# MuellerNico/DD2360-RayTracing

Measured on AMD Instinct MI355X. Metric: Msamples/s (W*H*spp/render_time) at 1200x800, 10000 spheres, higher is better.
Workload: dtype f32

## Files before the change

dd2360-raytracing_amd/csrc/rt_kernels.hip:

```cpp
#include <hip/hip_runtime.h>
#include <float.h>
#include "rt_device.h"
#include "rt_tuning.h"
#include "rt_sampling.h"
#include "rt_sched_keep.h"

#ifdef RT_TU_CONTRACT
#pragma clang fp contract(fast)
#else
#pragma clang fp contract(off)
#endif

namespace rt {
#ifdef RT_TU_CONTRACT
namespace fmac {
#endif

#define RT_DEV static __device__ __forceinline__

#include "rt_stats.h"

struct Rng { uint32_t d, v0, v1, v2, v3, v4; };

RT_DEV float rng_uniform(Rng& s) {
    const uint32_t t = s.v0 ^ (s.v0 >> 2);
    s.v0 = s.v1; s.v1 = s.v2; s.v2 = s.v3; s.v3 = s.v4;
    s.v4 = (s.v4 ^ (s.v4 << 4)) ^ (t ^ (t << 1));
    s.d += 362437u;
    return uniform_from_bits(s.d + s.v4);
}

RT_DEV void rng_seed(Rng& s, unsigned long long seed) {
    const uint32_t lo = (uint32_t)seed ^ 0xaad26b49u, hi = (uint32_t)(seed >> 32) ^ 0xf7dcefddu;
    const uint32_t t0 = 1099087573u * lo, t1 = 2591861531u * hi;
    s.d = 6615241u + t1 + t0;
    s.v0 = 123456789u + t0; s.v1 = 362436069u ^ t0; s.v2 = 521288629u + t1; s.v3 = 88675123u ^ t1; s.v4 = 5783321u + t0;
}

struct V3 { float x, y, z; };
RT_DEV float dot3(const V3& a, const V3& b) { return a.x * b.x + a.y * b.y + a.z * b.z; }

struct RayF { V3 o, d; };

RT_DEV float pow5(float x) { const double v = (double)x; const double v2 = v * v; return (float)((v2 * v2) * v); }

RT_DEV void sphere_test(const RayF& r, float a, float cx, float cy, float cz, float r2, int id, float& closest, int& best) {
    const float ocx = r.o.x - cx, ocy = r.o.y - cy, ocz = r.o.z - cz;
    const float b = ocx * r.d.x + ocy * r.d.y + ocz * r.d.z;
    const float c = (ocx * ocx + ocy * ocy + ocz * ocz) - r2;
    const float disc = b * b - a * c;
    if (disc > 0.0f) {
        const float sq = sqrtf(disc);
        float t = (-b - sq) / a;
        if (t < closest && t > 0.001f) { closest = t; best = id; }
        else {
            t = (-b + sq) / a;
            if (t < closest && t > 0.001f) { closest = t; best = id; }
        }
    }
}

RT_DEV bool ray_box(const RayF& r, float lox, float loy, float loz, float hix, float hiy, float hiz) {
    float tmin = (lox - r.o.x) / r.d.x;
    float tmax = (hix - r.o.x) / r.d.x;
    if (tmin > tmax) { const float t = tmin; tmin = tmax; tmax = t; }
    float tymin = (loy - r.o.y) / r.d.y;
    float tymax = (hiy - r.o.y) / r.d.y;
    if (tymin > tymax) { const float t = tymin; tymin = tymax; tymax = t; }
    if ((tmin > tymax) || (tymin > tmax)) return false;
    if (tymin > tmin) tmin = tymin;
    if (tymax < tmax) tmax = tymax;
    float tzmin = (loz - r.o.z) / r.d.z;
    float tzmax = (hiz - r.o.z) / r.d.z;
    if (tzmin > tzmax) { const float t = tzmin; tzmin = tzmax; tzmax = t; }
    if ((tmin > tzmax) || (tzmin > tmax)) return false;
    return true;
}

RT_DEV const RenderArgs* cold_args() {
    auto p = __builtin_amdgcn_kernarg_segment_ptr();
    asm volatile("" : "+s"(p));
    return (const RenderArgs*)p;
}

RT_DEV float bcast(float v, int l) { return __int_as_float(__builtin_amdgcn_readlane(__float_as_int(v), l)); }
template <int LG>
RT_DEV float group_min(float v) {
    const int inf = 0x7f800000;
    int x = __float_as_int(v);
#define RT_DPP_MIN(ctrl, rmask) x = __float_as_int(fminf(__int_as_float(x), __int_as_float(__builtin_amdgcn_update_dpp(inf, x, ctrl, rmask, 0xf, false))))
    RT_DPP_MIN(0x111, 0xf);
    RT_DPP_MIN(0x112, 0xf);
    RT_DPP_MIN(0x114, 0xf);
    RT_DPP_MIN(0x118, 0xf);
    if (LG >= 32) RT_DPP_MIN(0x142, 0xa);
    if (LG >= 64) RT_DPP_MIN(0x143, 0xc);
#undef RT_DPP_MIN
    const int q3 = __builtin_amdgcn_readlane(x, 63);
    if (LG == 64) return __int_as_float(q3);
    const int q1 = __builtin_amdgcn_readlane(x, 31);
    if (LG == 32) return __int_as_float((threadIdx.x & 32) ? q3 : q1);
    const int q0 = __builtin_amdgcn_readlane(x, 15), q2 = __builtin_amdgcn_readlane(x, 47);
    const int g = (threadIdx.x >> 4) & 3;
    return __int_as_float(g == 0 ? q0 : g == 1 ? q1 : g == 2 ? q2 : q3);
}
RT_DEV int wave_min_int(int x) {
    const int big = 0x7fffffff;
#define RT_DPP_MIN(ctrl, rmask) x = min(x, __builtin_amdgcn_update_dpp(big, x, ctrl, rmask, 0xf, false))
    RT_DPP_MIN(0x111, 0xf); RT_DPP_MIN(0x112, 0xf); RT_DPP_MIN(0x114, 0xf); RT_DPP_MIN(0x118, 0xf); RT_DPP_MIN(0x142, 0xa); RT_DPP_MIN(0x143, 0xc);
#undef RT_DPP_MIN
    return __builtin_amdgcn_readlane(x, 63);
}
RT_DEV int bcast(int v, int l) { return __builtin_amdgcn_readlane(v, l); }

RT_DEV float sphere_candidate(const RayF& r, float a, const float4 s) {
    const float ocx = r.o.x - s.x, ocy = r.o.y - s.y, ocz = r.o.z - s.z;
    const float b = ocx * r.d.x + ocy * r.d.y + ocz * r.d.z;
    const float c = (ocx * ocx + ocy * ocy + ocz * ocz) - s.w;
    const float disc = b * b - a * c;
    float cand = __builtin_inff();
    if (disc > 0.0f) {
        const float sq = sqrtf(disc);
        const float t1 = (-b - sq) / a;
        if (t1 > 0.001f) cand = t1;
        else {
            const float t2 = (-b + sq) / a;
            if (t2 > 0.001f) cand = t2;
        }
    }
    return cand;
}

RT_DEV void closest_list(const DevScene& S, const RayF& r, float a, bool live, float& closest, int& best) {
    const float4* __restrict__ hot = S.list_hot;
    const int n = S.n_list;
    unsigned long long todo = __ballot(live);
    if ((int)__popcll(todo) * RT_LIST_COOP_COST <= n) {
        const int lane = threadIdx.x & 63;
        while (todo != 0ull) {
            const int L = __ffsll((long long)todo) - 1;
            todo &= todo - 1ull;
            RayF q;
            q.o.x = bcast(r.o.x, L); q.o.y = bcast(r.o.y, L); q.o.z = bcast(r.o.z, L);
            q.d.x = bcast(r.d.x, L); q.d.y = bcast(r.d.y, L); q.d.z = bcast(r.d.z, L);
            const float qa = bcast(a, L);
            float my_t = FLT_MAX; int my_k = 0x7fffffff;
            for (int base = 0; base < n; base += 256) {
                float4 sv[4];
#pragma unroll
                for (int u = 0; u < 4; ++u) { const int k = base + u * 64 + lane; sv[u] = hot[k < n ? k : n - 1]; }
#pragma unroll
                for (int u = 0; u < 4; ++u) {
                    const int k = base + u * 64 + lane;
                    if (k < n) {
                        const float cand = sphere_candidate(q, qa, sv[u]);
                        if (cand < my_t) { my_t = cand; my_k = k; }
                    }
// ... 554 lines not shown
                bool anyhold = false;
#pragma unroll
                for (int k = 0; k < PB; ++k) {
                    const float ocx = S.q.o.x - s4[k].x, ocy = S.q.o.y - s4[k].y, ocz = S.q.o.z - s4[k].z;
                    const float b = ocx * S.q.d.x + ocy * S.q.d.y + ocz * S.q.d.z;
                    const float c = (ocx * ocx + ocy * ocy + ocz * ocz) - s4[k].w;
                    const float disc = b * b - S.a * c;
                    const float ab = fabsf(b);
                    const float Lm = __builtin_fmaf(ab, -1e-4f, -b) - S.abt, M = __builtin_fmaf(ab, -1e-4f, b) + S.atm;
                    const float P = fmaxf(Lm, M);
                    hold[k] = (unsigned)k < nb && disc > 0.0f && !(P > 0.0f && P * P > disc * 1.0003f);
                    hb[k] = b; hd[k] = disc;
                    anyhold = anyhold || hold[k];
                }
                if (__ballot(anyhold) != 0ull) {
#pragma unroll
                    for (int k = 0; k < PB; ++k) {
                        const unsigned long long hm = __ballot(hold[k]);
                        if (hm != 0ull) {
                            const unsigned slot = qn + __builtin_amdgcn_mbcnt_hi((unsigned)(hm >> 32), __builtin_amdgcn_mbcnt_lo((unsigned)hm, 0u));
                            if (hold[k]) {
                                STAT(st, ST_DISCPOS, 1);
                                const uint4 ce = make_uint4(__float_as_uint(hb[k]), __float_as_uint(hd[k]), he0 + (unsigned)k, (unsigned)S.owner);
                                if (slot < (unsigned)kWalkCand) L.cq[slot] = ce;
                                else pool_candidate(T, s_nodes, L, ce STAT_PASS);
                            }
                            qn += (unsigned)__popcll(hm);
                        }
                    }
                }
                S.cur += nb;
                if (qn >= (unsigned)RT_DENSE_DRAIN) pool_drain(T, s_nodes, L, lane, qn STAT_PASS);
            }
            pool_drain(T, s_nodes, L, lane, qn STAT_PASS);
            const unsigned long long k = L.key[lane];
            best_t = __uint_as_float((unsigned)(k >> 32)); best = (int)(unsigned)k;
            const unsigned tmask = lane < 32 ? L.tie_lo : L.tie_hi;
            if ((tmask >> (lane & 31)) & 1u) tie = true;
        }
        if (walking && best >= 0) walk_clip(W, A, best_t);
        walking = walking && W.i != W.iend;
        const int left = __popcll(__ballot(walking));
        if (left == 0) break;
        if (RT_QUORUM_DEN > 0 && nw0 >= RT_QUORUM_MIN && left * RT_QUORUM_DEN <= nw0) break;
    }
    W.walking = walking;
}

constexpr int kHotLarge = 8;
constexpr int kHotSlots = 1 + 3 * kHotLarge;
RT_DEV float4* hot_spheres(const float4* s_nodes, int n_nodes) { return (float4*)((WalkLds*)(s_nodes + n_nodes * 3) + 4); }
template <bool POOL>
RT_DEV void stage_tree_fp32(const DevScene& S, const DevTree& T, float4* s_nodes) {
    const int n4 = T.n_nodes * 3;
    for (int t = threadIdx.x; t < n4; t += 256) s_nodes[t] = T.nodes4[t];
    if (POOL) {
        float4* h = hot_spheres(s_nodes, T.n_nodes);
        const int nl = min(T.acc.n_large, kHotLarge);
        if (threadIdx.x == 0) h[0] = S.ground_valid ? S.list_hot[0] : make_float4(0.f, 0.f, 0.f, 0.f);
        if ((int)threadIdx.x < nl) h[1 + threadIdx.x] = T.acc.large_hot[threadIdx.x];
        if ((int)threadIdx.x < 2 * nl) h[1 + kHotLarge + threadIdx.x] = T.acc.large_brick[threadIdx.x];
    }
    __syncthreads();
}

struct TreeState { Walk W; float g_t; int g_id; bool tie, pending; unsigned work, cols; };
RT_DEV void tree_state_init(TreeState& ts) {
    ts.pending = false; ts.tie = false; ts.g_t = FLT_MAX; ts.g_id = -1; ts.work = 0u; ts.cols = 0u; ts.W.work = 0u; ts.W.cols = 0u;
    ts.W.walking = false; ts.W.i = 0; ts.W.iend = 0; ts.W.coff = 0; ts.W.om_c = 0.f; ts.W.on_c = 0.f; ts.W.slope = 0.f; ts.W.dm_c = 0.f; ts.W.fwd = true;
}

template <int COOPG>
RT_DEV void closest_tree(const DevScene& S, const DevTree& T, const float4* s_nodes, const RayF& r, float a, bool live, float& closest, int& best, TreeState& ts STAT_ARG) {
    const bool fresh = live && !ts.pending;
    STAT(st, ST_RAYS, fresh ? 1 : 0);
    if (fresh) { closest = FLT_MAX; best = -1; }
    if (S.ground_valid && fresh) {
        WPASS(WP_GROUND);
        const float4 g = COOPG != 1 ? hot_spheres(s_nodes, T.n_nodes)[0] : S.list_hot[0];
        int gb = -1;
        { const float ocx = r.o.x - g.x, ocy = r.o.y - g.y, ocz = r.o.z - g.z;
          const float b = ocx * r.d.x + ocy * r.d.y + ocz * r.d.z;
          const float c = (ocx * ocx + ocy * ocy + ocz * ocz) - g.w;
          if (__ballot(fresh && !(b > 0.0f && c > 0.0f)) != 0ull) sphere_test(r, a, g.x, g.y, g.z, g.w, 0, closest, gb); }
        if (gb == 0) best = 0;
    }
    RT_STATS_ONLY(
    const unsigned long long tG = TICK(); st.cyc[4] += tG;
    )
    bool slow = fresh;
    if (COOPG != 1 && T.acc.enabled) {
        const float zx = r.o.x, zy = r.o.y - 1.0f, zz = r.o.z;
        const bool fast = fresh && (a >= 9.094947e-13f) && (a <= 1.0995116e12f) && (r.d.x != 0.0f) && (r.d.z != 0.0f)
                          && (fabsf(r.d.y) >= 9.094947e-13f) && (zx * zx + zy * zy + zz * zz <= T.acc.zone2);
        slow = fresh && !fast;
        STAT(st, ST_FAST, fast ? 1 : 0); STAT(st, ST_SLOW, slow ? 1 : 0);
        if (fast) {
            ts.g_t = closest; ts.g_id = best; ts.tie = false;
            const float ra = __builtin_amdgcn_rcpf(a);
            for (int k = 0; k < T.acc.n_large; ++k) {
                const float4* hs = hot_spheres(s_nodes, T.n_nodes);
                const float4 sp = k < kHotLarge ? hs[1 + k] : T.acc.large_hot[k];
                WPASS(WP_LARGE_K);
                const float ocx = r.o.x - sp.x, ocy = r.o.y - sp.y, ocz = r.o.z - sp.z;
                const float b = ocx * r.d.x + ocy * r.d.y + ocz * r.d.z;
                const float c = (ocx * ocx + ocy * ocy + ocz * ocz) - sp.w;
                const float disc = b * b - a * c;
                if (disc > 0.0f) {
                    const float sqa = __builtin_amdgcn_sqrtf(disc);
                    const float m = 1e-4f * ((fabsf(b) + sqa) * ra) + 1e-6f;
                    const bool behind = (sqa - b) * ra + m < 0.001f;
                    const bool beyond = (-b - sqa) * ra - m > closest;
                    if (!behind && !beyond) {
                        WPASS(WP_LARGE_EXACT);
                        const float sq = sqrtf(disc);
                        float cand = __builtin_inff();
                        const float t1 = (-b - sq) / a;
                        if (t1 > 0.001f) cand = t1;
                        else { const float t2 = (-b + sq) / a; if (t2 > 0.001f) cand = t2; }
                        offer(T, s_nodes, r, cand, k < kHotLarge ? hs[1 + kHotLarge + 2 * k] : T.acc.large_brick[2 * k], k < kHotLarge ? hs[2 + kHotLarge + 2 * k] : T.acc.large_brick[2 * k + 1], closest, best, ts.tie STAT_PASS);
                    }
                }
            }
            WPASS(WP_SETUP);
            ts.W = walk_setup(T.acc, r, closest, best);
        }
        RT_STATS_ONLY(
        const unsigned long long tL = TICK(); st.cyc[5] += tL - tG;
        )
        const bool walker = fast || (live && ts.pending);
        const int nw = __popcll(__ballot(walker));
        if (nw > 0) {
            WalkLds& L = *((WalkLds*)(s_nodes + T.n_nodes * 3) + (threadIdx.x >> 6));
            Walk Wl = ts.W; Wl.walking = walker && ts.W.walking;
            float bt = walker ? closest : FLT_MAX; int bi = walker ? best : -1; bool tt = false;
            if (COOPG >= 4) walk_pool<RT_QUORUM_SPARSE>(T, s_nodes, L, r, a, Wl, bt, bi, tt STAT_PASS);
            else walk_pool_dense<RT_QUORUM_DENSE>(T, s_nodes, L, r, a, Wl, bt, bi, tt STAT_PASS);
            if (walker) { ts.work += Wl.work; ts.cols += Wl.cols; Wl.work = 0u; Wl.cols = 0u; ts.W = Wl; closest = bt; best = bi; ts.tie = ts.tie || tt; }
        }
        if (walker) {
            ts.pending = ts.W.walking;
            if (!ts.pending && ts.tie) { closest = ts.g_t; best = ts.g_id; slow = true; STAT(st, ST_TIE, 1); }
        }
    }
    RT_STATS_ONLY(
    const unsigned long long tS0 = TICK(); st.cyc[1] += tS0 - tG;
    )
    if (__ballot(slow) != 0ull) { WPASS(WP_SCAN); tree_scan(s_nodes, r, a, slow, closest, best); }
    RT_STATS_ONLY(
    st.cyc[3] += TICK() - tS0;
    )
}

RT_DEV V3 random_in_unit_sphere(Rng& s) {
    V3 p;
    do {
        WPASS(WP_REJ_ITER);
        const float x = rng_uniform(s); const float y = rng_uniform(s); const float z = rng_uniform(s);
        p.x = signed_unit(x); p.y = signed_unit(y); p.z = signed_unit(z);
    } while (p.x * p.x + p.y * p.y + p.z * p.z >= 1.0f);
    return p;
}

RT_DEV RayF primary_ray(const rt_camera& c, int i, int j, int max_x, int max_y, Rng& s) {
    const float u = ((float)i + rng_uniform(s)) / (float)max_x;
    const float v = ((float)j + rng_uniform(s)) / (float)max_y;
    float px, py;
    WPASS(WP_PRIMARY);
    do {
        WPASS(WP_DISK_ITER);
        const float x = rng_uniform(s); const float y = rng_uniform(s);
        px = signed_unit(x); py = signed_unit(y);
    } while (px * px + py * py + 0.0f >= 1.0f);
    const float rdx = c.lens_radius * px, rdy = c.lens_radius * py;
    RayF r;
    const float ox = rdx * c.u[0] + rdy * c.v[0], oy = rdx * c.u[1] + rdy * c.v[1], oz = rdx * c.u[2] + rdy * c.v[2];
    r.o.x = c.origin[0] + ox; r.o.y = c.origin[1] + oy; r.o.z = c.origin[2] + oz;
    r.d.x = (((c.lower_left_corner[0] + u * c.horizontal[0]) + v * c.vertical[0]) - c.origin[0]) - ox;
    r.d.y = (((c.lower_left_corner[1] + u * c.horizontal[1]) + v * c.vertical[1]) - c.origin[1]) - oy;
    r.d.z = (((c.lower_left_corner[2] + u * c.horizontal[2]) + v * c.vertical[2]) - c.origin[2]) - oz;
    return r;
}

RT_DEV bool scatter(const DevScene& S, int sphere, float t, RayF& r, V3& att, Rng& s) {
    const float4 g = S.shade[2 * sphere];
    const float4 m = S.shade[2 * sphere + 1];
    const int kind = S.kind8[sphere];
    V3 p, n;
    p.x = r.o.x + t * r.d.x; p.y = r.o.y + t * r.d.y; p.z = r.o.z + t * r.d.z;
    n.x = (p.x - g.x) / g.w; n.y = (p.y - g.y) / g.w; n.z = (p.z - g.z) / g.w;
    V3 q = {0.0f, 0.0f, 0.0f};
    WPASS(WP_SC_ANY);
    if (kind != RT_MAT_DIELECTRIC) q = random_in_unit_sphere(s);
    float len = 1.0f; V3 ud = {0.0f, 0.0f, 0.0f};
    if (kind != RT_MAT_LAMBERTIAN) {
        len = sqrtf(r.d.x * r.d.x + r.d.y * r.d.y + r.d.z * r.d.z);
        ud.x = r.d.x / len; ud.y = r.d.y / len; ud.z = r.d.z / len;
    }
    if (kind == RT_MAT_LAMBERTIAN) {
        WPASS(WP_SC_LAMB);
        const float tx = (p.x + n.x) + q.x, ty = (p.y + n.y) + q.y, tz = (p.z + n.z) + q.z;
        r.d.x = tx - p.x; r.d.y = ty - p.y; r.d.z = tz - p.z;
        r.o = p;
        att.x *= m.x; att.y *= m.y; att.z *= m.z;
        return true;
    }
    if (kind == RT_MAT_METAL) {
        WPASS(WP_SC_METAL);
        const float k = 2.0f * dot3(ud, n);
        const float rx = ud.x - k * n.x, ry = ud.y - k * n.y, rz = ud.z - k * n.z;
        r.d.x = rx + m.w * q.x; r.d.y = ry + m.w * q.y; r.d.z = rz + m.w * q.z;
        r.o = p;
        att.x *= m.x; att.y *= m.y; att.z *= m.z;
        return dot3(r.d, n) > 0.0f;
    }
    WPASS(WP_SC_DIEL);
    const float ri = m.w, inv_ri = m.x, r0sq = m.y, ri2 = m.z;
    const float dn = dot3(r.d, n);
    const float k = 2.0f * dn;
    const float rx = r.d.x - k * n.x, ry = r.d.y - k * n.y, rz = r.d.z - k * n.z;
    V3 on; float ni, cosine;
    if (dn > 0.0f) {
        on.x = -n.x; on.y = -n.y; on.z = -n.z; ni = ri;
        cosine = dn / len;
        cosine = sqrtf(1.0f - ri2 * (1.0f - cosine * cosine));
    } else {
        on = n; ni = inv_ri;
        cosine = -dn / len;
    }
    const V3 uv = ud;
    const float dt = dot3(uv, on);
    const float disc = 1.0f - ni * ni * (1.0f - dt * dt);
    float fx = 0.0f, fy = 0.0f, fz = 0.0f, reflect_prob;
    if (disc > 0.0f) {
        const float sq = sqrtf(disc);
        fx = ni * (uv.x - dt * on.x) - sq * on.x;
        fy = ni * (uv.y - dt * on.y) - sq * on.y;
        fz = ni * (uv.z - dt * on.z) - sq * on.z;
        const float r0 = r0sq;
        reflect_prob = r0 + (1.0f - r0) * pow5(1.0f - cosine);
    } else {
        reflect_prob = 1.0f;
    }
    r.o = p;
    if (rng_uniform(s) < reflect_prob) { r.d.x = rx; r.d.y = ry; r.d.z = rz; }
    else { r.d.x = fx; r.d.y = fy; r.d.z = fz; }
    return true;
}

RT_DEV V3 sky(const RayF& r, const V3& att) {
    WPASS(WP_SKY);
    const float len = sqrtf(r.d.x * r.d.x + r.d.y * r.d.y + r.d.z * r.d.z);
    const float uy = r.d.y / len;
    const float t = 0.5f * (uy + 1.0f);
    const float omt = 1.0f - t;
    V3 c;
    c.x = att.x * (omt + t * 0.5f);
    c.y = att.y * (omt + t * 0.7f);
    c.z = att.z * (omt + t * 1.0f);
    return c;
}

#ifndef RT_TU_LIST
__global__ __launch_bounds__(256) void k_render_init(rt_rand_state* rand_state, int max_x, int max_y, int tiles_x, int part, int nparts, long long begin, long long end, long long n_local_tiles) {
    const int lane = threadIdx.x & 63;
    const long long local_tile = (long long)blockIdx.x * 4 + (threadIdx.x >> 6);
    if (local_tile >= n_local_tiles) return;
    const long long tile = part_tile(local_tile, part, nparts, begin, end);
    const int tx = (int)(tile % tiles_x), ty = (int)(tile / tiles_x);
    const int i = tx * 8 + (lane & 7), j = ty * 8 + (lane >> 3);
    const bool inside = (i < max_x) && (j < max_y);
    const bool whole = part_whole(nparts, begin, end);
    if (whole && !inside) return;
    const long long idx = whole ? (long long)j * max_x + i : local_tile * 64 + lane;
    const int pixel_index = j * max_x + i;
    Rng s; rng_seed(s, 1984ull + (unsigned long long)(long long)pixel_index);
    rt_rand_state out;
    out.d = s.d; out.v[0] = s.v0; out.v[1] = s.v1; out.v[2] = s.v2; out.v[3] = s.v3; out.v[4] = s.v4;
    out.boxmuller_flag = 0; out.boxmuller_flag_double = 0; out.boxmuller_extra = 0.f; out.pad_ = 0; out.boxmuller_extra_double = 0.0;
    rand_state[idx] = out;
}
#endif

template <bool TREE, int MODE, int COOPG>
__global__ __launch_bounds__(256, RT_RENDER_WAVES) void k_render(RenderArgs A) {
    extern __shared__ float4 s_nodes[];
    if (TREE) stage_tree_fp32<COOPG != 1>(A.scene, A.tree, s_nodes);
    const int lane = threadIdx.x & 63;
    const long long n_slots = (MODE == 2 && A.ad_list) ? (long long)*A.ad_count : A.n_local_tiles * 64;
    const int ns = (MODE != 1) ? A.ns : 1;

    const long long n_waves = (long long)gridDim.x * 4;
    long long slot = 0;
    int i = 0, j = 0; long long idx = 0;
    unsigned int iters = 0;
    bool is_long = false;
    bool is_med = false;
    bool retired = false;
    bool thin = false;
    bool thin_counted = false;
    bool long_done = false;
    const unsigned int n_long_raw = A.long_list ? A.queue[2] : 0u, n_solo_raw = A.long_list ? A.queue[4] : 0u;
    const bool use_long = (n_long_raw + n_solo_raw) != 0u && (long long)(n_long_raw + n_solo_raw) * 64 <= n_slots;
    const unsigned int n_long = use_long ? n_long_raw : 0u, n_solo = use_long ? n_solo_raw : 0u;
    bool solo = false, solo_done = false;
    Rng s = {0, 0, 0, 0, 0, 0};
    V3 col = {0.0f, 0.0f, 0.0f};
    V3 att = {1.0f, 1.0f, 1.0f};
    float sum_l = 0.0f, sum_q = 0.0f;
    RayF r; r.o = {0.f, 0.f, 0.f}; r.d = {0.f, 1.f, 0.f};
    int sample = 0, depth = 0;
    bool live = false;
    RT_STATS_ONLY(
    unsigned int pix_iters = 0;
    unsigned long long pix_t0 = 0;
    )

    constexpr bool kChunked = MODE == 1;
    constexpr long long kProgOwn = RT_PROG_OWN;
    const long long first_free = (kChunked && kProgOwn > 0 && n_waves * kProgOwn <= n_slots) ? n_waves * kProgOwn : 0;
    long long pool_next = 0, pool_end = 0;
    if (kChunked && first_free > 0) { pool_next = ((long long)blockIdx.x * 4 + (threadIdx.x >> 6)) * kProgOwn; pool_end = pool_next + kProgOwn; }
    auto take_slot = [&]() -> long long {
        return first_free + (long long)atomicAdd(cold_args()->queue, 1u);
    };
    auto begin_pixel = [&]() {
        live = false;
        const RenderArgs& A = *cold_args();
#ifdef RT_ONLY_LANE
        if (lane != RT_ONLY_LANE) return;
#endif
        iters = 0; is_long = false; is_med = false;
        while (slot < n_slots) {
            if constexpr (MODE == 2) {
                if (A.ad_list) {
                    const unsigned int pid = A.ad_list[slot];
                    idx = (long long)pid;
                    if (part_whole(A.nparts, A.tile_begin, A.tile_end)) { i = (int)(pid % (unsigned int)A.max_x); j = (int)(pid / (unsigned int)A.max_x); }
                    else {
                        const long long tile = part_tile((long long)(pid >> 6), A.part, A.nparts, A.tile_begin, A.tile_end);
                        const int tx = (int)(tile % A.tiles_x), ty = (int)(tile / A.tiles_x);
                        i = tx * 8 + (int)(pid & 7u); j = ty * 8 + (int)((pid >> 3) & 7u);
                    }
                    live = true;
                    break;
                }
            }
            long long local_tile; int l;
            const long long tail0 = (MODE != 1 && A.tail_list) ? (long long)A.queue[kQueueThr + 2] : 0;
            const long long head = tail0 > 0 ? (long long)A.queue[kQueueThr + 3] : 0;
            if (tail0 > 0 && (slot < head || slot >= tail0 - 1 + head)) {
                const bool from_end = A.queue[kQueueThr + 5] != 0u;
                const long long n_tail = n_slots - (tail0 - 1);
                const long long k = slot < head ? (from_end ? n_tail - head + slot : slot) : (from_end ? slot - (tail0 - 1) - head : slot - (tail0 - 1));
                const unsigned int pid = A.tail_list[k];
                local_tile = (long long)(pid >> 6); l = (int)(pid & 63u);
            } else {
                constexpr int kIl = COOPG == 2 ? RT_INTERLEAVE_DENSE : (COOPG == 5 ? RT_INTERLEAVE_SOLO : RT_INTERLEAVE);
                static_assert(kIl > 0 && 64 % kIl == 0, "RT_INTERLEAVE, RT_INTERLEAVE_DENSE and RT_INTERLEAVE_SOLO must divide 64 (the tail starts on a multiple of 64 tiles)");
                const long long ms = slot - head;
                const long long blk = ms / (64 * kIl);
                const long long tiles_in_blk = (A.n_local_tiles - blk * kIl) < kIl ? (A.n_local_tiles - blk * kIl) : kIl;
                const long long within = ms % (64 * kIl);
                const long long rank = blk * kIl + within % tiles_in_blk;
                l = (int)(within / tiles_in_blk);
                local_tile = A.order ? (long long)A.order[rank] : rank;
            }
            const long long tile = part_tile(local_tile, A.part, A.nparts, A.tile_begin, A.tile_end);
            const int tx = (int)(tile % A.tiles_x), ty = (int)(tile / A.tiles_x);
            i = tx * 8 + (l & 7); j = ty * 8 + (l >> 3);
            const bool taken = use_long && A.long_flag[local_tile * 64 + l];
            if (i < A.max_x && j < A.max_y && !taken) {
                idx = part_whole(A.nparts, A.tile_begin, A.tile_end) ? (long long)j * A.max_x + i : local_tile * 64 + l;
                live = true;
                RT_STATS_ONLY(
                pix_t0 = __builtin_amdgcn_s_memrealtime();
                )
                break;
            }
            slot = take_slot();
        }
        if (!live) retired = true;
        if (live) {
            const rt_rand_state* st = A.rand_state + idx;
            s.d = st->d; s.v0 = st->v[0]; s.v1 = st->v[1]; s.v2 = st->v[2]; s.v3 = st->v[3]; s.v4 = st->v[4];
            col = {0.0f, 0.0f, 0.0f}; att = {1.0f, 1.0f, 1.0f}; sample = 0; depth = 0;
            if constexpr (MODE == 2) {
                sum_l = 0.0f; sum_q = 0.0f;
                if (A.ad_list) {
                    const float* f = (const float*)A.fb + idx * 3;
                    col.x = f[0]; col.y = f[1]; col.z = f[2]; sum_l = A.ad_sl[idx]; sum_q = A.ad_q[idx];
                }
            }
            r = primary_ray(A.scene.cam, i, j, A.max_x, A.max_y, s);
        }
    };
    auto begin_long_pixel = [&](bool from_solo) -> bool {
        if (!use_long || (from_solo ? solo_done : long_done)) return false;
        const RenderArgs& A = *cold_args();
        long long pid;
        if (from_solo) {
            const unsigned int h = atomicAdd(A.queue + 5, 1u);
            if (h >= n_solo) { solo_done = true; return false; }
            pid = (long long)A.long_list[n_slots - 1 - (long long)h];
        } else {
            const unsigned int h = atomicAdd(A.queue + 3, 1u);
            if (h >= n_long) { long_done = true; return false; }
            const unsigned int stride = n_long % 257u ? 257u : (n_long % 263u ? 263u : 269u);
            pid = (long long)A.long_list[(unsigned int)(((unsigned long long)h * stride) % n_long)];
        }
        const long long local_tile = pid >> 6;
        const int l = (int)(pid & 63);
        const long long tile = part_tile(local_tile, A.part, A.nparts, A.tile_begin, A.tile_end);
        const int tx = (int)(tile % A.tiles_x), ty = (int)(tile / A.tiles_x);
        i = tx * 8 + (l & 7); j = ty * 8 + (l >> 3);
        idx = part_whole(A.nparts, A.tile_begin, A.tile_end) ? (long long)j * A.max_x + i : pid;
        live = true; iters = 0; is_long = true;
        RT_STATS_ONLY(
        pix_t0 = __builtin_amdgcn_s_memrealtime();
        )
        const rt_rand_state* st = A.rand_state + idx;
        s.d = st->d; s.v0 = st->v[0]; s.v1 = st->v[1]; s.v2 = st->v[2]; s.v3 = st->v[3]; s.v4 = st->v[4];
        col = {0.0f, 0.0f, 0.0f}; att = {1.0f, 1.0f, 1.0f}; sample = 0; depth = 0;
        if constexpr (MODE == 2) { sum_l = 0.0f; sum_q = 0.0f; }
        r = primary_ray(A.scene.cam, i, j, A.max_x, A.max_y, s);
        return true;
    };
    auto end_pixel = [&]() {
        const RenderArgs& A = *cold_args();
        rt_rand_state* st_out = A.rand_state + idx;
        st_out->d = s.d; st_out->v[0] = s.v0; st_out->v[1] = s.v1; st_out->v[2] = s.v2; st_out->v[3] = s.v3; st_out->v[4] = s.v4;
        float* fb = (float*)A.fb + idx * 3;
        if constexpr (MODE == 2) {
            fb[0] = col.x; fb[1] = col.y; fb[2] = col.z;
            A.ad_sl[idx] = sum_l; A.ad_q[idx] = sum_q;
        } else if (MODE == 0) {
            const float k = (float)(1.0 / (double)(float)A.ns);
            col.x *= k; col.y *= k; col.z *= k;
            fb[0] = sqrtf(col.x); fb[1] = sqrtf(col.y); fb[2] = sqrtf(col.z);
            RT_STATS_ONLY(
            fb[0] = (float)pix_iters; fb[1] = (float)((__builtin_amdgcn_s_memrealtime() >> 4) & 0xffffffull); fb[2] = (float)((pix_t0 >> 4) & 0xffffffull);
            )
        } else {
            if (A.ns == 1) { fb[0] = col.x; fb[1] = col.y; fb[2] = col.z; }
            else { fb[0] += col.x; fb[1] += col.y; fb[2] += col.z; }
        }
    };
    RT_STATS_ONLY(
    Stats st; for (int q = 0; q < ST_N; ++q) st.c[q] = 0;
    for (int q = 0; q < 8; ++q) st.cyc[q] = 0;
    const unsigned long long tK0 = TICK(), rK0 = __builtin_amdgcn_s_memrealtime();
    unsigned int dbg_thin_iters = 0, dbg_long = 0;
    unsigned long long th[4] = {0, 0, 0, 0};
    unsigned long long dbg_thin_cyc = 0, dbg_thin_closest = 0, dbg_thin1_cyc = 0; unsigned int dbg_thin1_iters = 0; unsigned long long dbg_t_prev = TICK();
    )
    constexpr bool kSolo = TREE && COOPG == 5;
    if (kSolo && lane == 0 && begin_long_pixel(true)) solo = true;
    if (__ballot(live) == 0ull && lane < RT_LONG_PER_WAVE) begin_long_pixel(false);
    if (__ballot(live) != 0ull) { thin = true; __builtin_amdgcn_s_setprio(3); }

    const unsigned int thin_cap = (unsigned int)(n_waves / RT_THIN_CAP_DEN);
    float closest = FLT_MAX; int best = -1;
    TreeState ts; tree_state_init(ts);
    while (true) {
        const unsigned long long m_live = __ballot(live);
        const unsigned long long m_long = __ballot(live && is_long);
        if (!thin && m_long != 0ull) {
            unsigned int prev = 0;
            if (lane == 0) prev = atomicAdd(cold_args()->queue + 1, 1u);
            prev = __builtin_amdgcn_readfirstlane(prev);
            if (prev < thin_cap) { thin = true; thin_counted = true; __builtin_amdgcn_s_setprio(3); }
            else { if (lane == 0) atomicSub(cold_args()->queue + 1, 1u); is_long = false; }
        } else if (thin && m_long == 0ull) {
            thin = false; __builtin_amdgcn_s_setprio(0);
            if (thin_counted && lane == 0) atomicSub(A.queue + 1, 1u);
            thin_counted = false;
        }
        if (RT_MED_RATE > 0 && !thin) { if (__ballot(live && is_med) != 0ull) __builtin_amdgcn_s_setprio(1); else __builtin_amdgcn_s_setprio(0); }
        if (!thin) {
            if (kChunked) {
                const bool need = !live && !retired;
                const unsigned long long mneed = __ballot(need);
                if (mneed != 0ull) {
                    const long long n = (long long)__popcll(mneed);
                    const long long left = pool_end - pool_next;
                    const long long rank = (long long)__builtin_amdgcn_mbcnt_hi((unsigned)(mneed >> 32), __builtin_amdgcn_mbcnt_lo((unsigned)mneed, 0u));
                    long long fresh = 0;
                    if (n > left) {
                        unsigned int b = 0;
                        if (lane == 0) b = atomicAdd(cold_args()->queue, 64u);
                        fresh = first_free + (long long)__builtin_amdgcn_readfirstlane(b);
                    }
                    if (need) slot = rank < left ? pool_next + rank : fresh + (rank - left);
                    if (n > left) { pool_next = fresh + (n - left); pool_end = fresh + 64; } else pool_next += n;
                    if (need) begin_pixel();
                }
            } else if (!live && !retired) { slot = take_slot(); begin_pixel(); }
        }
        if (__ballot(live) == 0ull) break;
        (void)m_live;
        STAT(st, ST_LOOP_ITERS_WAVE, 1);
        RT_STATS_ONLY(
        { const unsigned long long now = TICK(); const int nl2 = __popcll(__ballot(live));
          if (thin) { ++dbg_thin_iters; dbg_thin_cyc += now - dbg_t_prev; if (nl2 <= 2) { ++dbg_thin1_iters; dbg_thin1_cyc += now - dbg_t_prev; } }
          dbg_t_prev = now; }
        )
        RT_STATS_ONLY(
        { const int nl = __popcll(__ballot(live)); STAT(st, nl >= 56 ? ST_LIVE_GE56 : nl >= 32 ? ST_LIVE_32 : nl >= 8 ? ST_LIVE_8 : ST_LIVE_LT8, 1);
          WPASS_CLASS(nl >= 56 ? 0 : nl >= 32 ? 1 : nl >= 8 ? 2 : 3); }
        )
        const float a = dot3(r.d, r.d);
        if (!TREE) { closest = FLT_MAX; best = -1; }
        RT_STATS_ONLY(
        const unsigned long long tC0 = TICK();
        const unsigned long long c4_ = st.cyc[4], c5_ = st.cyc[5], c1_ = st.cyc[1], c3_ = st.cyc[3];
        const bool thin12 = thin && __popcll(__ballot(live)) <= 2;
        )
        if (TREE) closest_tree<COOPG>(A.scene, A.tree, s_nodes, r, a, live, closest, best, ts STAT_PASS);
        else closest_list(A.scene, r, a, live, closest, best);
        RT_STATS_ONLY(
        const unsigned long long tC1 = TICK(); st.cyc[0] += tC1 - tC0; st.cyc[2] += tC0; if (thin) dbg_thin_closest += tC1 - tC0;
        if (TREE && thin12) { th[0] += (st.cyc[4] - c4_) - tC0; th[1] += st.cyc[5] - c5_; th[2] += (st.cyc[1] - c1_) - (st.cyc[5] - c5_); th[3] += st.cyc[3] - c3_; }
        if (live) { ++pix_iters; }
        )
        if (live && !(TREE && ts.pending)) {
            ++iters;
            bool done;
            float lum = 0.0f;
            if (best >= 0) {
                const bool cont = scatter(cold_args()->scene, best, closest, r, att, s);
                ++depth;
                done = !cont || depth >= 50;
            } else {
                const V3 c = sky(r, att);
                col.x += c.x; col.y += c.y; col.z += c.z;
                if constexpr (MODE == 2) lum = (c.x + c.y) + c.z;
                done = true;
            }
            if (done) {
                if constexpr (MODE == 2) { sum_l += lum; sum_q += lum * lum; }
                (void)lum;
                ++sample; depth = 0; att = {1.0f, 1.0f, 1.0f};
                if (sample < ns) {
                    { const RenderArgs& C = *cold_args(); r = primary_ray(C.scene.cam, i, j, C.max_x, C.max_y, s); }
                    bool now_long = false;
                    if ((sample & (RT_LONG_CHECK - 1)) == 0 && sample + 8 <= ns) {
                        const unsigned int long_thr = MODE != 1 ? cold_args()->queue[kQueueThr] : 0u;
                        now_long = iters >= (unsigned int)((COOPG == 2 ? RT_LONG_RATE_DENSE : RT_LONG_RATE) * sample) ||
                                   (long_thr != 0u && (unsigned long long)iters * (unsigned int)ns >= (unsigned long long)long_thr * (unsigned int)sample);
                    }
                    if (now_long) {
                        RT_STATS_ONLY(
                        if (!is_long) ++dbg_long;
                        )
                        is_long = true;
                    }
                    else if (RT_MED_RATE > 0 && (sample & 7) == 0 && iters >= (unsigned int)(RT_MED_RATE * sample)) is_med = true;
                } else {
                    WPASS(WP_ENDPIX);
                    end_pixel();
                    RT_STATS_ONLY(
                    pix_iters = 0;
                    )
                    STAT(st, ST_SWITCHES, 1);
                    live = false; is_long = false; is_med = false;
                    if (kSolo && solo && begin_long_pixel(true)) {  }
                    else if (lane < RT_LONG_PER_WAVE && begin_long_pixel(false)) { solo = false;  }
                }
            }
        }
    }

    RT_STATS_ONLY(
    for (int q = 0; q < ST_N; ++q) {
        const bool wave_level = (q == ST_LOOP_ITERS_WAVE || (q >= ST_LIVE_GE56 && q <= ST_LIVE_LT8));
        const bool lane_max = (q == ST_A_ITERS_WAVE || q == ST_B_ROUNDS_WAVE);
        if (lane_max) { int m = (int)st.c[q]; for (int off = 32; off > 0; off >>= 1) m = max(m, __shfl_xor(m, off)); if (lane == 0) atomicAdd(&g_stats[q], (unsigned long long)m); }
        else if (st.c[q] && (!wave_level || lane == 0)) atomicAdd(&g_stats[q], (unsigned long long)st.c[q]);
    }
    { int nl = (int)dbg_long; for (int off = 32; off > 0; off >>= 1) nl += __shfl_xor(nl, off); dbg_long = (unsigned int)nl; }
    if (lane == 0) {
        const long long wv = (long long)blockIdx.x * 4 + (threadIdx.x >> 6);
        if (wv < 8192) {
            g_wave_dbg[wv * 4 + 0] = __builtin_amdgcn_s_memrealtime();
            g_wave_dbg[wv * 4 + 1] = st.c[ST_LOOP_ITERS_WAVE]; g_wave_dbg[wv * 4 + 2] = dbg_thin_iters; g_wave_dbg[wv * 4 + 3] = dbg_long;
            atomicAdd(&g_stats[TH_GROUND], th[0]); atomicAdd(&g_stats[TH_LARGE_SETUP], th[1]); atomicAdd(&g_stats[TH_WALK], th[2]); atomicAdd(&g_stats[TH_SCAN], th[3]);
            atomicAdd(&g_stats[ST_SPARE0], dbg_thin_cyc); atomicAdd(&g_stats[ST_SPARE1], dbg_thin_closest); atomicAdd(&g_stats[ST_SPARE2], dbg_thin1_cyc); atomicAdd(&g_stats[ST_SPARE3], (unsigned long long)dbg_thin1_iters); atomicAdd(&g_stats[ST_SPARE4], (unsigned long long)dbg_thin_iters);
        }
        atomicAdd(&g_stats[ST_SAMPLES], 1ull);
        const unsigned long long tot = TICK() - tK0;
        atomicAdd(&g_stats[ST_CYC_TOTAL], tot);
        atomicAdd(&g_stats[ST_CYC_CLOSEST], st.cyc[0]); atomicAdd(&g_stats[ST_CYC_WALK_A], st.cyc[1]); atomicAdd(&g_stats[ST_CYC_WALK_B], st.cyc[4] - st.cyc[2]);
        atomicAdd(&g_stats[ST_CYC_SCAN], st.cyc[3]); atomicAdd(&g_stats[ST_CYC_SHADE], tot - st.cyc[0]); atomicAdd(&g_stats[ST_SPARE4 + 1], st.cyc[5]); atomicAdd(&g_stats[ST_SPARE4 + 2], st.cyc[6]);
        atomicAdd(&g_stats[ST_REALTIME], __builtin_amdgcn_s_memrealtime() - rK0);
    }
    )
}

#if !defined(RT_TU_LIST) && !defined(RT_TU_CONTRACT)
__device__ __forceinline__ bool adapt_rule(float S, float Q, int k, float rel_error, float floor_lum) {
    const float nk = (float)k;
    const float d = nk * Q - S * S;
    const float nf = nk * floor_lum;
    const float m = S > nf ? S : nf;
    const float tt = rel_error * rel_error;
    return rel_error > 0.f && d <= (tt * (nk - 1.f)) * (m * m);
}
__device__ __forceinline__ bool adapt_in_frame(long long t, const AdaptFrame& fr) {
    const long long tile = part_tile(t >> 6, fr.part, fr.nparts, fr.tile_begin, fr.tile_end);
    const int tx = (int)(tile % fr.tiles_x), ty = (int)(tile / fr.tiles_x);
    return tx * 8 + (int)(t & 7) < fr.max_x && ty * 8 + (int)((t >> 3) & 7) < fr.max_y;
}
__device__ __forceinline__ void adapt_append(bool active, unsigned int pid, unsigned int* list_out, unsigned int* count_out) {
    const unsigned long long mask = __ballot(active);
    if (mask != 0ull) {
        unsigned int base = 0;
        if ((threadIdx.x & 63) == 0) base = atomicAdd(count_out, (unsigned int)__popcll(mask));
        base = __shfl(base, 0);
        const unsigned int rank = __builtin_amdgcn_mbcnt_hi((unsigned)(mask >> 32), __builtin_amdgcn_mbcnt_lo((unsigned)mask, 0u));
        if (active) list_out[base + rank] = pid;
    }
}
template <bool KEEP>
__device__ __forceinline__ void adapt_check(float* __restrict__ fb, const float* __restrict__ sl, const float* __restrict__ q,
                                            const unsigned int* __restrict__ list_in, const unsigned int* __restrict__ count_in, long long n_all,
                                            unsigned int* __restrict__ list_out, unsigned int* __restrict__ count_out, int32_t* __restrict__ spp,
                                            int k, int last, float rel_error, float floor_lum, const AdaptFrame& fr, const AdaptState& keep) {
    const long long t = (long long)blockIdx.x * 256 + threadIdx.x;
    const long long n = count_in ? (long long)*count_in : n_all;
    bool active = false;
    unsigned int pid = 0;
    bool inside = true;
    if (!list_in && t < n && !part_whole(fr.nparts, fr.tile_begin, fr.tile_end)) {
        const long long tile = part_tile(t >> 6, fr.part, fr.nparts, fr.tile_begin, fr.tile_end);
        const int tx = (int)(tile % fr.tiles_x), ty = (int)(tile / fr.tiles_x);
        inside = tx * 8 + (int)(t & 7) < fr.max_x && ty * 8 + (int)((t >> 3) & 7) < fr.max_y;
    }
    if (t < n && inside) {
        pid = list_in ? list_in[t] : (unsigned int)t;
        bool stop = last != 0;
        if (!stop) stop = adapt_rule(sl[pid], q[pid], k, rel_error, floor_lum);
        if (stop) {
            float* f = fb + (size_t)pid * 3;
            const float kk = (float)(1.0 / (double)(float)k);
            if constexpr (KEEP) {
                float* s = keep.rgb + (size_t)pid * 3;
                s[0] = f[0]; s[1] = f[1]; s[2] = f[2];
                keep.k[pid] = k;
            }
            f[0] = sqrtf(f[0] * kk); f[1] = sqrtf(f[1] * kk); f[2] = sqrtf(f[2] * kk);
            if (spp) spp[pid] = k;
        } else {
            active = true;
        }
    }
    adapt_append(active, pid, list_out, count_out);
}
__global__ __launch_bounds__(256) void k_adapt_check(float* __restrict__ fb, const float* __restrict__ sl, const float* __restrict__ q,
                                                     const unsigned int* __restrict__ list_in, const unsigned int* __restrict__ count_in, long long n_all,
                                                     unsigned int* __restrict__ list_out, unsigned int* __restrict__ count_out, int32_t* __restrict__ spp,
                                                     int k, int last, float rel_error, float floor_lum, AdaptFrame fr) {
    adapt_check<false>(fb, sl, q, list_in, count_in, n_all, list_out, count_out, spp, k, last, rel_error, floor_lum, fr, AdaptState{});
}
__global__ __launch_bounds__(256) void k_adapt_check_keep(float* __restrict__ fb, AdaptState s,
                                                          const unsigned int* __restrict__ list_in, const unsigned int* __restrict__ count_in, long long n_all,
                                                          unsigned int* __restrict__ list_out, unsigned int* __restrict__ count_out, int32_t* __restrict__ spp,
                                                          int k, int last, float rel_error, float floor_lum, AdaptFrame fr) {
    adapt_check<true>(fb, s.sl, s.q, list_in, count_in, n_all, list_out, count_out, spp, k, last, rel_error, floor_lum, fr, s);
}

__global__ __launch_bounds__(256) void k_adapt_refine_seed(float* __restrict__ fb, AdaptState s, long long n_all, unsigned int* __restrict__ list_out,
                                                           unsigned int* __restrict__ count_out, int32_t* __restrict__ spp,
                                                           int max_spp, float rel_error, float floor_lum, AdaptFrame fr) {
    const long long t = (long long)blockIdx.x * 256 + threadIdx.x;
    bool active = false;
    const unsigned int pid = (unsigned int)t;
    if (t < n_all && (part_whole(fr.nparts, fr.tile_begin, fr.tile_end) || adapt_in_frame(t, fr))) {
        const int k = s.k[pid];
        const float* S = s.rgb + (size_t)pid * 3;
        float* f = fb + (size_t)pid * 3;
        if (k >= max_spp || adapt_rule(s.sl[pid], s.q[pid], k, rel_error, floor_lum)) {
            const float kk = (float)(1.0 / (double)(float)k);
            f[0] = sqrtf(S[0] * kk); f[1] = sqrtf(S[1] * kk); f[2] = sqrtf(S[2] * kk);
            if (spp) spp[pid] = k;
        } else {
            f[0] = S[0]; f[1] = S[1]; f[2] = S[2];
            active = true;
        }
    }
    adapt_append(active, pid, list_out, count_out);
}
__global__ __launch_bounds__(256) void k_adapt_refine_check(float* __restrict__ fb, AdaptState s,
                                                            const unsigned int* __restrict__ list_in, const unsigned int* __restrict__ count_in,
                                                            unsigned int* __restrict__ list_out, unsigned int* __restrict__ count_out, int32_t* __restrict__ spp,
                                                            int batch, int max_spp, float rel_error, float floor_lum) {
    const long long t = (long long)blockIdx.x * 256 + threadIdx.x;
    bool active = false;
// ... 703 lines not shown
```

dd2360-raytracing_amd/csrc/rt_stats.h:

```cpp
#pragma once
#ifdef RT_STATS
enum { ST_RAYS, ST_FAST, ST_SLOW, ST_TIE, ST_COLS, ST_TESTS, ST_DISCPOS, ST_OFFERS, ST_ELIG, ST_ELIG_NODES, ST_A_ITERS_WAVE, ST_B_ROUNDS_WAVE,
       ST_LOOP_ITERS_WAVE, ST_A_LANE_STEPS, ST_B_LANES, ST_SAMPLES, ST_LIVE_GE56, ST_LIVE_32, ST_LIVE_8, ST_LIVE_LT8, ST_SWITCHES,
       ST_CYC_TOTAL, ST_CYC_CLOSEST, ST_CYC_WALK_A, ST_CYC_WALK_B, ST_CYC_SCAN, ST_CYC_SHADE, ST_REALTIME,
       ST_SPARE0, ST_SPARE1, ST_SPARE2, ST_SPARE3, ST_SPARE4, ST_SPARE5, ST_SPARE6,
       WP_GROUND, WP_LARGE_K, WP_LARGE_EXACT, WP_OFFER_NODE, WP_OFFER_RAYBOX, WP_ELIG_FN, WP_ELIG_LIST, WP_SETUP, WP_A_COL, WP_A_BATCH, WP_A_HOLD,
       WP_B_OFFER, WP_B_CLIP, WP_COOP_CHUNK, WP_SCAN, WP_SC_ANY, WP_SC_LAMB, WP_SC_METAL, WP_SC_DIEL, WP_REJ_ITER, WP_PRIMARY, WP_DISK_ITER, WP_SKY, WP_ENDPIX,
       TH_GROUND, TH_LARGE_SETUP, TH_WALK, TH_SCAN, ST_N };
#ifdef RT_STATS_LIGHT
#define TICK() 0ull
#else
#define TICK() ((unsigned long long)__builtin_amdgcn_s_memtime())
#endif
__device__ unsigned long long g_stats[ST_N];
__device__ int g_pilot_dbg[1 << 20];
__device__ unsigned long long g_wave_dbg[8192 * 4];
struct Stats { unsigned int c[ST_N]; unsigned long long cyc[8]; };
#ifdef RT_STATS_LIGHT
#define STAT(st, k, v) ((void)0)
#else
#define STAT(st, k, v) ((st).c[k] += (v))
#endif
constexpr int kWpBlocks = WP_ENDPIX - WP_GROUND + 1;
__device__ unsigned long long g_wp_cls[4 * kWpBlocks];
#ifdef RT_STATS_WPASS
__shared__ int s_wp_cls[4];
#define WPASS(k) do { const int l_ = (int)(threadIdx.x & 63); if (__builtin_amdgcn_readfirstlane(l_) == l_) { atomicAdd(&g_stats[k], 1ull); \
    atomicAdd(&g_wp_cls[(s_wp_cls[(threadIdx.x >> 6) & 3] & 3) * kWpBlocks + ((k) - WP_GROUND)], 1ull); } } while (0)
#define WPASS_CLASS(c) do { const int l_ = (int)(threadIdx.x & 63); if (__builtin_amdgcn_readfirstlane(l_) == l_) s_wp_cls[(threadIdx.x >> 6) & 3] = (c); } while (0)
#else
#define WPASS(k) ((void)0)
#define WPASS_CLASS(c) ((void)0)
#endif
#define STAT_ARG , Stats& st
#define STAT_PASS , st
#define RT_STATS_ONLY(...) __VA_ARGS__
#define RT_STATS_READERS \
hipError_t read_pilot_dbg(int* out, int n) { return hipMemcpyFromSymbol(out, HIP_SYMBOL(g_pilot_dbg), sizeof(int) * (size_t)(n < (1 << 20) ? n : (1 << 20))); } \
hipError_t read_wave_dbg(unsigned long long* out) { return hipMemcpyFromSymbol(out, HIP_SYMBOL(g_wave_dbg), sizeof(unsigned long long) * 8192 * 4); } \
hipError_t read_wp_classes(unsigned long long* out, int reset) { \
    hipError_t e = hipMemcpyFromSymbol(out, HIP_SYMBOL(g_wp_cls), sizeof(unsigned long long) * 4 * kWpBlocks); \
    if (e != hipSuccess) return e; \
    if (reset) { unsigned long long z[4 * kWpBlocks] = {0}; e = hipMemcpyToSymbol(HIP_SYMBOL(g_wp_cls), z, sizeof(z)); } \
    return e; \
} \
hipError_t read_stats(unsigned long long* out, int reset) { \
    hipError_t e = hipMemcpyFromSymbol(out, HIP_SYMBOL(g_stats), sizeof(unsigned long long) * ST_N); \
    if (e != hipSuccess) return e; \
    if (reset) { unsigned long long z[ST_N] = {0}; e = hipMemcpyToSymbol(HIP_SYMBOL(g_stats), z, sizeof(z)); } \
    return e; \
}
#else
#define STAT(st, k, v) ((void)0)
#define WPASS(k) ((void)0)
#define WPASS_CLASS(c) ((void)0)
#define STAT_ARG
#define STAT_PASS
#define RT_STATS_ONLY(...)
#define RT_STATS_READERS
#endif
```

Measured before the change: 4771.

## Merge divergent rejection-sampling loops into a shared wave-level sampling state machine

Restructures the shading step so that the unit-sphere rejection loop for opaque scatter, the pixel jitter and the lens-disk rejection loop for the next primary ray all run through one shared loop driven by a small mode state machine. Lanes at different stages can now draw RNG samples in the same wave iteration instead of running several separately divergent loops. Sky shading reuses a unit-direction computation shared with the glass path, and the tile-slot index math switches from 64-bit to 32-bit division. The cost is more live registers and extra control logic in the hot loop, with RNG consumption order kept the same per lane.

```diff
diff --git a/dd2360-raytracing_amd/csrc/rt_kernels.hip b/dd2360-raytracing_amd/csrc/rt_kernels.hip
--- a/dd2360-raytracing_amd/csrc/rt_kernels.hip
+++ b/dd2360-raytracing_amd/csrc/rt_kernels.hip
@@ -3,6 +3,7 @@
 #include "rt_device.h"
 #include "rt_tuning.h"
 #include "rt_sampling.h"
+#include "rt_sample_merge.h"
 #include "rt_sched_keep.h"
 
 #ifdef RT_TU_CONTRACT
@@ -863,26 +864,44 @@
     )
 }
 
+RT_DEV bool unit_point(float x, float y, float z, float& px, float& py, float& pz) {
+    px = signed_unit(x); py = signed_unit(y); pz = signed_unit(z);
+    return !(px * px + py * py + pz * pz >= 1.0f);
+}
+
 RT_DEV V3 random_in_unit_sphere(Rng& s) {
     V3 p;
+    bool ok;
     do {
         WPASS(WP_REJ_ITER);
         const float x = rng_uniform(s); const float y = rng_uniform(s); const float z = rng_uniform(s);
-        p.x = signed_unit(x); p.y = signed_unit(y); p.z = signed_unit(z);
-    } while (p.x * p.x + p.y * p.y + p.z * p.z >= 1.0f);
+        ok = unit_point(x, y, z, p.x, p.y, p.z);
+    } while (!ok);
     return p;
 }
 
-RT_DEV RayF primary_ray(const rt_camera& c, int i, int j, int max_x, int max_y, Rng& s) {
-    const float u = ((float)i + rng_uniform(s)) / (float)max_x;
-    const float v = ((float)j + rng_uniform(s)) / (float)max_y;
-    float px, py;
-    WPASS(WP_PRIMARY);
+RT_DEV void primary_jitter(float x, float y, int i, int j, int max_x, int max_y, float& u, float& v) {
+    u = ((float)i + x) / (float)max_x;
+    v = ((float)j + y) / (float)max_y;
+}
+RT_DEV void random_in_unit_disk(Rng& s, float& px, float& py) {
+    float pz; bool ok;
     do {
         WPASS(WP_DISK_ITER);
         const float x = rng_uniform(s); const float y = rng_uniform(s);
-        px = signed_unit(x); py = signed_unit(y);
-    } while (px * px + py * py + 0.0f >= 1.0f);
+        ok = unit_point(x, y, 0.5f, px, py, pz);
+    } while (!ok);
+}
+RT_DEV int sampling_pass(Rng& s, int mode, int i, int j, int max_x, int max_y, float& u, float& v, float& px, float& py, float& pz) {
+    const float x = rng_uniform(s); const float y = rng_uniform(s);
+    float z = 0.5f;
+    if (mode == SM_SPHERE) z = rng_uniform(s);
+    bool ok = false;
+    if (mode == SM_JITTER) primary_jitter(x, y, i, j, max_x, max_y, u, v);
+    else ok = unit_point(x, y, z, px, py, pz);
+    return sm_after_pass(mode, ok);
+}
+RT_DEV RayF primary_lens(const rt_camera& c, float u, float v, float px, float py) {
     const float rdx = c.lens_radius * px, rdy = c.lens_radius * py;
     RayF r;
     const float ox = rdx * c.u[0] + rdy * c.v[0], oy = rdx * c.u[1] + rdy * c.v[1], oz = rdx * c.u[2] + rdy * c.v[2];
@@ -892,23 +911,32 @@
     r.d.z = (((c.lower_left_corner[2] + u * c.horizontal[2]) + v * c.vertical[2]) - c.origin[2]) - oz;
     return r;
 }
-
-RT_DEV bool scatter(const DevScene& S, int sphere, float t, RayF& r, V3& att, Rng& s) {
+RT_DEV RayF primary_ray(const rt_camera& c, int i, int j, int max_x, int max_y, Rng& s) {
+    const float x = rng_uniform(s); const float y = rng_uniform(s);
+    float u, v, px, py;
+    primary_jitter(x, y, i, j, max_x, max_y, u, v);
+    WPASS(WP_PRIMARY);
+    random_in_unit_disk(s, px, py);
+    return primary_lens(c, u, v, px, py);
+}
+
+struct Surf { V3 p, n; float4 m; int kind; };
+RT_DEV Surf scatter_head(const DevScene& S, int sphere, float t, const RayF& r) {
     const float4 g = S.shade[2 * sphere];
-    const float4 m = S.shade[2 * sphere + 1];
-    const int kind = S.kind8[sphere];
-    V3 p, n;
-    p.x = r.o.x + t * r.d.x; p.y = r.o.y + t * r.d.y; p.z = r.o.z + t * r.d.z;
-    n.x = (p.x - g.x) / g.w; n.y = (p.y - g.y) / g.w; n.z = (p.z - g.z) / g.w;
-    V3 q = {0.0f, 0.0f, 0.0f};
-    WPASS(WP_SC_ANY);
-    if (kind != RT_MAT_DIELECTRIC) q = random_in_unit_sphere(s);
-    float len = 1.0f; V3 ud = {0.0f, 0.0f, 0.0f};
-    if (kind != RT_MAT_LAMBERTIAN) {
-        len = sqrtf(r.d.x * r.d.x + r.d.y * r.d.y + r.d.z * r.d.z);
-        ud.x = r.d.x / len; ud.y = r.d.y / len; ud.z = r.d.z / len;
-    }
-    if (kind == RT_MAT_LAMBERTIAN) {
+    Surf h;
+    h.m = S.shade[2 * sphere + 1];
+    h.kind = S.kind8[sphere];
+    h.p.x = r.o.x + t * r.d.x; h.p.y = r.o.y + t * r.d.y; h.p.z = r.o.z + t * r.d.z;
+    h.n.x = (h.p.x - g.x) / g.w; h.n.y = (h.p.y - g.y) / g.w; h.n.z = (h.p.z - g.z) / g.w;
+    return h;
+}
+RT_DEV void unit_direction(const RayF& r, float& len, V3& ud) {
+    len = sqrtf(r.d.x * r.d.x + r.d.y * r.d.y + r.d.z * r.d.z);
+    ud.x = r.d.x / len; ud.y = r.d.y / len; ud.z = r.d.z / len;
+}
+RT_DEV bool scatter_opaque(const Surf& h, const V3& q, const V3& ud, RayF& r, V3& att) {
+    const V3 p = h.p, n = h.n; const float4 m = h.m;
+    if (h.kind == RT_MAT_LAMBERTIAN) {
         WPASS(WP_SC_LAMB);
         const float tx = (p.x + n.x) + q.x, ty = (p.y + n.y) + q.y, tz = (p.z + n.z) + q.z;
         r.d.x = tx - p.x; r.d.y = ty - p.y; r.d.z = tz - p.z;
@@ -916,16 +944,17 @@
         att.x *= m.x; att.y *= m.y; att.z *= m.z;
         return true;
     }
-    if (kind == RT_MAT_METAL) {
-        WPASS(WP_SC_METAL);
-        const float k = 2.0f * dot3(ud, n);
-        const float rx = ud.x - k * n.x, ry = ud.y - k * n.y, rz = ud.z - k * n.z;
-        r.d.x = rx + m.w * q.x; r.d.y = ry + m.w * q.y; r.d.z = rz + m.w * q.z;
-        r.o = p;
-        att.x *= m.x; att.y *= m.y; att.z *= m.z;
-        return dot3(r.d, n) > 0.0f;
-    }
+    WPASS(WP_SC_METAL);
+    const float k = 2.0f * dot3(ud, n);
+    const float rx = ud.x - k * n.x, ry = ud.y - k * n.y, rz = ud.z - k * n.z;
+    r.d.x = rx + m.w * q.x; r.d.y = ry + m.w * q.y; r.d.z = rz + m.w * q.z;
+    r.o = p;
+    att.x *= m.x; att.y *= m.y; att.z *= m.z;
+    return dot3(r.d, n) > 0.0f;
+}
+RT_DEV void scatter_glass(const Surf& h, float len, const V3& ud, RayF& r, Rng& s) {
     WPASS(WP_SC_DIEL);
+    const V3 p = h.p, n = h.n; const float4 m = h.m;
     const float ri = m.w, inv_ri = m.x, r0sq = m.y, ri2 = m.z;
     const float dn = dot3(r.d, n);
     const float k = 2.0f * dn;
@@ -956,13 +985,21 @@
     r.o = p;
     if (rng_uniform(s) < reflect_prob) { r.d.x = rx; r.d.y = ry; r.d.z = rz; }
     else { r.d.x = fx; r.d.y = fy; r.d.z = fz; }
+}
+RT_DEV bool scatter(const DevScene& S, int sphere, float t, RayF& r, V3& att, Rng& s) {
+    const Surf h = scatter_head(S, sphere, t, r);
+    V3 q = {0.0f, 0.0f, 0.0f};
+    WPASS(WP_SC_ANY);
+    if (h.kind != RT_MAT_DIELECTRIC) q = random_in_unit_sphere(s);
+    float len = 1.0f; V3 ud = {0.0f, 0.0f, 0.0f};
+    if (h.kind != RT_MAT_LAMBERTIAN) unit_direction(r, len, ud);
+    if (h.kind != RT_MAT_DIELECTRIC) return scatter_opaque(h, q, ud, r, att);
+    scatter_glass(h, len, ud, r, s);
     return true;
 }
 
-RT_DEV V3 sky(const RayF& r, const V3& att) {
+RT_DEV V3 sky(float uy, const V3& att) {
     WPASS(WP_SKY);
-    const float len = sqrtf(r.d.x * r.d.x + r.d.y * r.d.y + r.d.z * r.d.z);
-    const float uy = r.d.y / len;
     const float t = 0.5f * (uy + 1.0f);
     const float omt = 1.0f - t;
     V3 c;
@@ -1072,9 +1109,11 @@
                 const long long ms = slot - head;
                 const long long blk = ms / (64 * kIl);
                 const long long tiles_in_blk = (A.n_local_tiles - blk * kIl) < kIl ? (A.n_local_tiles - blk * kIl) : kIl;
-                const long long within = ms % (64 * kIl);
-                const long long rank = blk * kIl + within % tiles_in_blk;
-                l = (int)(within / tiles_in_blk);
+                const unsigned int within = (unsigned int)(ms % (64 * kIl));
+                const unsigned int tib = (unsigned int)tiles_in_blk;
+                const unsigned int lq = within / tib;
+                const long long rank = blk * kIl + (long long)(within - lq * tib);
+                l = (int)lq;
                 local_tile = A.order ? (long long)A.order[rank] : rank;
             }
             const long long tile = part_tile(local_tile, A.part, A.nparts, A.tile_begin, A.tile_end);
@@ -1236,24 +1275,58 @@
         )
         if (live && !(TREE && ts.pending)) {
             ++iters;
-            bool done;
+            const bool hit = best >= 0;
+            const bool more = sample + 1 < ns;
+            bool done = !hit;
             float lum = 0.0f;
-            if (best >= 0) {
-                const bool cont = scatter(cold_args()->scene, best, closest, r, att, s);
-                ++depth;
-                done = !cont || depth >= 50;
-            } else {
-                const V3 c = sky(r, att);
+            Surf h; h.kind = RT_MAT_DIELECTRIC; h.p = {0.0f, 0.0f, 0.0f}; h.n = {0.0f, 0.0f, 0.0f}; h.m = make_float4(0.0f, 0.0f, 0.0f, 0.0f);
+            WPASS(WP_SC_ANY);
+            if (hit) h = scatter_head(cold_args()->scene, best, closest, r);
+            const bool opaque = hit && h.kind != RT_MAT_DIELECTRIC;
+            float len = 1.0f; V3 ud = {0.0f, 0.0f, 0.0f};
+            if (!hit || h.kind != RT_MAT_LAMBERTIAN) unit_direction(r, len, ud);
+            if (!hit) {
+                const V3 c = sky(ud.y, att);
                 col.x += c.x; col.y += c.y; col.z += c.z;
                 if constexpr (MODE == 2) lum = (c.x + c.y) + c.z;
-                done = true;
+            } else if (!opaque) {
+                scatter_glass(h, len, ud, r, s);
+                ++depth;
+                done = sm_path_ended(true, depth);
+            }
+            int mode = sm_enter(opaque, done, more);
+            bool tail = opaque;
+            float u = 0.0f, v = 0.0f, px = 0.0f, py = 0.0f, pz = 0.0f;
+#pragma unroll 1
+            for (int trip = 0; trip < 2; ++trip) {
+                RT_STATS_ONLY(
+                if (trip == 1) WPASS(WP_MERGE_TRIP2);
+                )
+                while (mode != SM_NONE) {
+                    RT_STATS_ONLY(
+                    WPASS(WP_MERGE_PASS);
+                    if (__ballot(mode == SM_SPHERE) != 0ull) WPASS(WP_REJ_ITER);
+                    if (__ballot(mode != SM_SPHERE) != 0ull) WPASS(WP_DISK_ITER);
+                    )
+                    { const RenderArgs& C = *cold_args(); mode = sampling_pass(s, mode, i, j, C.max_x, C.max_y, u, v, px, py, pz); }
+                }
+                if (tail) {
+                    tail = false;
+                    const V3 q = {px, py, pz};
+                    const bool cont = scatter_opaque(h, q, ud, r, att);
+                    ++depth;
+                    done = sm_path_ended(cont, depth);
+                    mode = sm_after_tail(done, more);
+                }
+                if (__ballot(mode != SM_NONE) == 0ull) break;
             }
             if (done) {
                 if constexpr (MODE == 2) { sum_l += lum; sum_q += lum * lum; }
                 (void)lum;
                 ++sample; depth = 0; att = {1.0f, 1.0f, 1.0f};
                 if (sample < ns) {
-                    { const RenderArgs& C = *cold_args(); r = primary_ray(C.scene.cam, i, j, C.max_x, C.max_y, s); }
+                    WPASS(WP_PRIMARY);
+                    r = primary_lens(cold_args()->scene.cam, u, v, px, py);
                     bool now_long = false;
                     if ((sample & (RT_LONG_CHECK - 1)) == 0 && sample + 8 <= ns) {
                         const unsigned int long_thr = MODE != 1 ? cold_args()->queue[kQueueThr] : 0u;
diff --git a/dd2360-raytracing_amd/csrc/rt_sample_merge.h b/dd2360-raytracing_amd/csrc/rt_sample_merge.h
--- /dev/null
+++ b/dd2360-raytracing_amd/csrc/rt_sample_merge.h
@@ -0,0 +1,24 @@
+#pragma once
+
+#if defined(__HIPCC__) || defined(__CUDACC__)
+#define RT_SM_FN static __host__ __device__ __forceinline__
+#else
+#define RT_SM_FN static inline
+#endif
+
+namespace rt {
+
+enum { SM_NONE = 0, SM_SPHERE = 1, SM_JITTER = 2, SM_DISK = 3 };
+constexpr int kMaxDepth = 50;
+
+RT_SM_FN bool sm_path_ended(bool cont, int depth_after) { return !cont || depth_after >= kMaxDepth; }
+
+RT_SM_FN int sm_enter(bool hit_opaque, bool ended, bool more) { return hit_opaque ? SM_SPHERE : ((ended && more) ? SM_JITTER : SM_NONE); }
+
+RT_SM_FN int sm_draws(int mode) { return mode == SM_SPHERE ? 3 : (mode == SM_NONE ? 0 : 2); }
+
+RT_SM_FN int sm_after_pass(int mode, bool accepted) { return mode == SM_JITTER ? SM_DISK : (accepted ? SM_NONE : mode); }
+
+RT_SM_FN int sm_after_tail(bool ended, bool more) { return (ended && more) ? SM_JITTER : SM_NONE; }
+
+}
diff --git a/dd2360-raytracing_amd/csrc/rt_stats.h b/dd2360-raytracing_amd/csrc/rt_stats.h
--- a/dd2360-raytracing_amd/csrc/rt_stats.h
+++ b/dd2360-raytracing_amd/csrc/rt_stats.h
@@ -6,6 +6,7 @@
        ST_SPARE0, ST_SPARE1, ST_SPARE2, ST_SPARE3, ST_SPARE4, ST_SPARE5, ST_SPARE6,
        WP_GROUND, WP_LARGE_K, WP_LARGE_EXACT, WP_OFFER_NODE, WP_OFFER_RAYBOX, WP_ELIG_FN, WP_ELIG_LIST, WP_SETUP, WP_A_COL, WP_A_BATCH, WP_A_HOLD,
        WP_B_OFFER, WP_B_CLIP, WP_COOP_CHUNK, WP_SCAN, WP_SC_ANY, WP_SC_LAMB, WP_SC_METAL, WP_SC_DIEL, WP_REJ_ITER, WP_PRIMARY, WP_DISK_ITER, WP_SKY, WP_ENDPIX,
+       WP_MERGE_PASS, WP_MERGE_TRIP2,
        TH_GROUND, TH_LARGE_SETUP, TH_WALK, TH_SCAN, ST_N };
 #ifdef RT_STATS_LIGHT
 #define TICK() 0ull
@@ -21,7 +22,7 @@
 #else
 #define STAT(st, k, v) ((st).c[k] += (v))
 #endif
-constexpr int kWpBlocks = WP_ENDPIX - WP_GROUND + 1;
+constexpr int kWpBlocks = WP_MERGE_TRIP2 - WP_GROUND + 1;
 __device__ unsigned long long g_wp_cls[4 * kWpBlocks];
 #ifdef RT_STATS_WPASS
 __shared__ int s_wp_cls[4];
```

After: 4477. -6.2%, worse.
